# TheoCoombes/ClipCap

Measured on AMD Instinct MI355X. Metric: train samples/sec (512-d prefix, 40-tok caption), higher is better.
Workload: dtype bf16; 1 GPU; BASELINE configs[1]: TransformerMapper(8L,P=L=10,H=8)+frozen GPT-2-small; per_gpu_batch=256, global_batch=256, encoder_dim=512, train_language_model=False, parallelism=dp1

## Files before the change

clipcap_amd/csrc/attention.hip:

```cpp
#include "kernels.h"

namespace CC_NS {

__device__ __forceinline__ void load_head_rows(float* dst, int hdp, const act_t* src, size_t ld, int S, int hd) {
    const int c8n = hd >> 3;
    for (int idx = threadIdx.x; idx < S * c8n; idx += blockDim.x) {
        const int r = idx / c8n, c = idx % c8n;
        float f[8];
        act_ld8(src + (size_t)r * ld + c * 8, f);
        float* d = dst + r * hdp + c * 8;
        *reinterpret_cast<float4*>(d) = make_float4(f[0], f[1], f[2], f[3]);
        *reinterpret_cast<float4*>(d + 4) = make_float4(f[4], f[5], f[6], f[7]);
    }
}

template <auto Kernel, class... Args>
static void attn_launch(dim3 grid, dim3 block, size_t sh, hipStream_t st, const Args&... args) {
    if (sh > 64 * 1024) (void)hipFuncSetAttribute((const void*)Kernel, hipFuncAttributeMaxDynamicSharedMemorySize, (int)sh);
    hipLaunchKernelGGL(Kernel, grid, block, sh, st, args...);
}
#define ATTN_LADDER(LAUNCH) { if (drop.thresh) { LAUNCH(true, true); } else if (causal) { LAUNCH(true, false); } else { LAUNCH(false, false); } }

__device__ __forceinline__ unsigned attn_drop_idx(int b, int H, int h, int S, int q, int k) { return ((unsigned)(b * H + h) * S + q) * S + k; }
template <bool CAUSAL>
// ... 443 lines not shown
#pragma unroll
        for (int r = 0; r < 16; r++) acc[r] = 0.f;
        if (kind == 0) {
            const int jn = CAUSAL ? blk + 1 : NBLK;
            for (int j = 0; j < jn; j++)
#pragma unroll
                for (int t = 0; t < 2; t++) {
                    const op16x8 a_h = frag_row_p(Dh + (blk * 32 + l31) * LDP + j * 32, t, half), a_l = frag_row_p(Dl + (blk * 32 + l31) * LDP + j * 32, t, half);
                    const op16x8 b_h = frag_tr_p<LD>(Kh + j * 32 * LD, nb, t, lane), b_l = frag_tr_p<LD>(Kl + j * 32 * LD, nb, t, lane);
                    CC_MFMA3(a_h, a_l, b_h, b_l, acc)
                }
        } else {
            const op16_t* Ah = kind == 1 ? Dh : Ph, *Al = kind == 1 ? Dl : Pl, *Bh = kind == 1 ? Qh : Oh, *Bl = kind == 1 ? Ql : Ol;
            for (int i = CAUSAL ? blk : 0; i < NBLK; i++)
#pragma unroll
                for (int t = 0; t < 2; t++) {
                    const op16x8 a_h = frag_tr_p<LDP>(Ah + i * 32 * LDP, blk, t, lane), a_l = frag_tr_p<LDP>(Al + i * 32 * LDP, blk, t, lane);
                    const op16x8 b_h = frag_tr_p<LD>(Bh + i * 32 * LD, nb, t, lane), b_l = frag_tr_p<LD>(Bl + i * 32 * LD, nb, t, lane);
                    CC_MFMA3(a_h, a_l, b_h, b_l, acc)
                }
        }
        const int d = nb * 32 + l31;
        if (img) {
            const int odd = lane & 1;
            op16_t* r3 = reinterpret_cast<op16_t*>(dqkv) + (size_t)b * S * 9 * D + kind * D + h * HD + (d & ~1);
#pragma unroll
            for (int rp = 0; rp < 8; rp++) {
                const float v0 = acc[2 * rp], v1 = acc[2 * rp + 1];
                const float got = __shfl_xor(odd ? v0 : v1, 1, 64);
                const float a0 = odd ? got : v0, a1 = odd ? v1 : got;
                const int row = blk * 32 + ((2 * rp) & 3) + 8 * ((2 * rp) >> 2) + 4 * half + odd;
                const unsigned hi = pack2op(a0, a1);
                float h0, h1;
                unpack2(hi, h0, h1);
                const unsigned lo = pack2op(a0 - h0, a1 - h1);
                if (row < S) {
                    op16_t* o3 = r3 + (size_t)row * 9 * D;
                    *reinterpret_cast<unsigned*>(o3) = hi;
                    *reinterpret_cast<unsigned*>(o3 + 3 * D) = hi;
                    *reinterpret_cast<unsigned*>(o3 + 6 * D) = lo;
                }
            }
        } else {
            float* o1 = dqkv + (size_t)b * S * rs + kind * D + h * HD + d;
#pragma unroll
            for (int r = 0; r < 16; r++) {
                const int row = blk * 32 + (r & 3) + 8 * (r >> 2) + 4 * half;
                if (row < S) o1[(size_t)row * rs] = acc[r];
            }
        }
    }
    __syncthreads();
    }
}
template <int HD, int NBLK>
static int attn_bwd_m3_launch(const float* qkv, const float* dout, const float* lse, int B, int S, int H, bool causal, float* dqkv, hipStream_t st,
                              Drop drop, int img) {
    typedef AttM3<HD, NBLK> G;
    const float scale = 1.0f / sqrtf((float)HD);
    static int ncu = 0;
    if (!ncu) {
        int dev = 0;
        hipDeviceProp_t pr;
        if (hipGetDevice(&dev) != hipSuccess || hipGetDeviceProperties(&pr, dev) != hipSuccess) return CC_ERR_STATE;
        ncu = pr.multiProcessorCount;
    }
    const int per_cu = (int)((size_t)160 * 1024 / G::lds);
    const dim3 grid(min(B * H, ncu * max(1, per_cu))), blk(64 * G::NW);
    if (drop.thresh && !causal) return CC_ERR_SHAPE;
#define CC_L(C, DR) attn_launch<k_attn_bwd_m3<HD, NBLK, C, DR>>(grid, blk, G::lds, st, qkv, dout, lse, B, S, H, scale, dqkv, drop, img)
    ATTN_LADDER(CC_L)
#undef CC_L
    return hipGetLastError() == hipSuccess ? CC_OK : CC_ERR_LAUNCH;
}
static bool attn_x3mfma_on();
static bool attn_bwd_m3_ok(int S, int hd) { return attn_x3mfma_on() && (hd == 64 || hd == 96) && S > 0 && S <= 64; }
static bool attn_x3mfma_on() {
    static const bool on = !(cc_lab_env("CC_ATTN_X3MFMA") && atoi(cc_lab_env("CC_ATTN_X3MFMA")) == 0) && !cc_lab_env("CC_ATTN_F32MFMA");
    return on;
}
#endif

#if CC_OP != 2
template <int HD, bool CAUSAL, bool DROP = false>
__global__ __launch_bounds__(256, HD == 64 ? 3 : 2) void k_attn_fwd_mfma(const op16_t* __restrict__ qkv, int B, int S, int H, float scale,
                                                       op16_t* __restrict__ out, float* __restrict__ lse_out, Drop drop = Drop()) {
    constexpr int KK = HD / 16, NB = HD / 32, C8 = HD / 8;
    __shared__ __attribute__((aligned(16))) op16_t vsm[4][32 * AttLd<HD>::v];
    const int lane = threadIdx.x & 63, wave = threadIdx.x >> 6;
    const int nqb = (S + 31) >> 5;
    const int item = blockIdx.x * 4 + wave;
    if (item >= B * H * nqb) return;
    const int qb = item % nqb, h = (item / nqb) % H, b = item / (nqb * H);
    const int D = H * HD;
    const size_t rs = (size_t)3 * D;
    const op16_t* base = qkv + (size_t)b * S * rs + h * HD;
    const int half = lane >> 5, q = qb * 32 + (lane & 31);
    op16_t* vs = vsm[wave];

    op16x8 qf[KK];
#pragma unroll
    for (int kk = 0; kk < KK; kk++) {
        qf[kk] = load_frag(base + (size_t)min(q, S - 1) * rs + kk * 16 + half * 8, q < S);
    }
    f32x16 o[NB];
    acc_zero(o);
    float m = -INFINITY, l = 0.f;
    const int nkb = CAUSAL ? qb + 1 : nqb;
    uint4 kq[KK], vq[HD / 16];
    auto fetch = [&](int kb, uint4 (&kd)[KK], uint4 (&vd)[HD / 16]) {
        const int key = kb * 32 + (lane & 31);
#pragma unroll
        for (int kk = 0; kk < KK; kk++) {
            kd[kk] = *reinterpret_cast<const uint4*>(base + D + (size_t)min(key, S - 1) * rs + kk * 16 + half * 8);
            if (key >= S) kd[kk] = make_uint4(0, 0, 0, 0);
        }
#pragma unroll
        for (int c = 0; c < HD / 16; c++) {
            const int idx = lane + 64 * c;
            const int vk = idx / C8, vc = idx % C8;
            vd[c] = *reinterpret_cast<const uint4*>(base + 2 * D + (size_t)min(kb * 32 + vk, S - 1) * rs + vc * 8);
            if (kb * 32 + vk >= S) vd[c] = make_uint4(0, 0, 0, 0);
        }
    };
    fetch(0, kq, vq);
    for (int kb = 0; kb < nkb; kb++) {
        uint4 kn[KK], vn[HD / 16];
        fetch(kb + 1, kn, vn);
        f32x16 s;
        acc_zero(s);
#pragma unroll
        for (int kk = 0; kk < KK; kk++) s = CC_MFMA_32x32x16(__builtin_bit_cast(op16x8, kq[kk]), qf[kk], s);
#pragma unroll
        for (int c = 0; c < HD / 16; c++) {
            const int idx = lane + 64 * c;
            *reinterpret_cast<uint4*>(vs + (idx / C8) * AttLd<HD>::v + (idx % C8) * 8) = vq[c];
        }
        float mx = -INFINITY;
#pragma unroll
        for (int r = 0; r < 16; r++) {
            const int kr = kb * 32 + c_row(r, half);
            const bool ok = kr < S && (!CAUSAL || kr <= q);
            s[r] = ok ? s[r] * scale : -INFINITY;
            mx = fmaxf(mx, s[r]);
        }
        mx = fmaxf(mx, __shfl_xor(mx, 32, 64));
        const float m_new = fmaxf(m, mx);
        const float alpha = (m == -INFINITY) ? 0.f : __expf(m - m_new);
        float p[16], ps = 0.f;
#pragma unroll
        for (int r = 0; r < 16; r++) {
            p[r] = (m_new == -INFINITY) ? 0.f : __expf(s[r] - m_new);
            ps += p[r];
        }
        ps += __shfl_xor(ps, 32, 64);
        l = l * alpha + ps;
        m = m_new;
#pragma unroll
        for (int nb = 0; nb < NB; nb++)
#pragma unroll
            for (int r = 0; r < 16; r++) o[nb][r] *= alpha;
        if (DROP) {
            const unsigned rowbase = attn_drop_idx(b, H, h, S, min(q, S - 1), 0);
#pragma unroll
            for (int r = 0; r < 16; r++) p[r] *= drop_mul(drop, rowbase + min(kb * 32 + c_row(r, half), S - 1));
        }
        op16x8 pf[2];
#pragma unroll
        for (int t = 0; t < 2; t++) pf[t] = pack_frag(p + t * 8);
#pragma unroll
        for (int t = 0; t < 2; t++)
#pragma unroll
            for (int nb = 0; nb < NB; nb++) o[nb] = CC_MFMA_32x32x16(frag_tr<HD>(vs, nb, t, lane), pf[t], o[nb]);
#pragma unroll
        for (int kk = 0; kk < KK; kk++) kq[kk] = kn[kk];
#pragma unroll
        for (int c = 0; c < HD / 16; c++) vq[c] = vn[c];
    }
    if (q < S) {
        const float inv = l > 0.f ? 1.f / l : 0.f;
        op16_t* orow = out + ((size_t)b * S + q) * D + h * HD;
        store_acc_row<NB, true>(orow, o, half, inv);
        if (half == 0 && lse_out) lse_out[((size_t)b * H + h) * S + q] = m + __logf(l);
    }
}

template <int HD>
static int attn_fwd_mfma_launch(const op16_t* qkv, int B, int S, int H, bool causal, op16_t* out, float* lse, hipStream_t st, Drop drop) {
    const int items = B * H * ((S + 31) / 32);
    const float scale = 1.0f / sqrtf((float)HD);
    if (drop.thresh && !causal) return CC_ERR_SHAPE;
#define CC_L(C, DR) attn_launch<k_attn_fwd_mfma<HD, C, DR>>(dim3((items + 3) / 4), dim3(256), 0, st, qkv, B, S, H, scale, out, lse, drop)
    ATTN_LADDER(CC_L)
#undef CC_L
    return hipGetLastError() == hipSuccess ? CC_OK : CC_ERR_LAUNCH;
}


template <int HD, bool CAUSAL, bool DROP = false>
__global__ __launch_bounds__(256, HD == 64 ? 2 : 1) void k_attn_bwd_dkv(const op16_t* __restrict__ qkv, const op16_t* __restrict__ dout,
                                                      const float* __restrict__ lse, const float* __restrict__ delta, int B, int S, int H,
                                                      float scale, op16_t* __restrict__ dqkv, Drop drop = Drop()) {
    constexpr int KK = HD / 16, NB = HD / 32;
    __shared__ __attribute__((aligned(16))) op16_t qsm[4][32 * AttLd<HD>::v];
    __shared__ __attribute__((aligned(16))) op16_t dsm[4][32 * AttLd<HD>::v];
    __shared__ __attribute__((aligned(16))) float ldsm[4][64];
    const int lane = threadIdx.x & 63, wave = threadIdx.x >> 6;
    const int nblk = (S + 31) >> 5;
    const int item = blockIdx.x * 4 + wave;
    if (item >= B * H * nblk) return;
    const int j = item % nblk, h = (item / nblk) % H, b = item / (nblk * H);
    const int D = H * HD;
    const size_t rs = (size_t)3 * D;
    const op16_t* base = qkv + (size_t)b * S * rs + h * HD;
    const op16_t* dbase = dout + (size_t)b * S * D + h * HD;
    const float* lrow = lse + ((size_t)b * H + h) * S;
    const float* drow = delta + ((size_t)b * H + h) * S;
    const int half = lane >> 5, key = j * 32 + (lane & 31);
    op16x8 kf[KK], vf[KK];
#pragma unroll
    for (int kk = 0; kk < KK; kk++) {
        kf[kk] = load_frag(base + D + (size_t)min(key, S - 1) * rs + kk * 16 + half * 8, key < S);
        vf[kk] = load_frag(base + 2 * D + (size_t)min(key, S - 1) * rs + kk * 16 + half * 8, key < S);
    }
    f32x16 dk[NB], dv[NB];
#pragma unroll
    for (int nb = 0; nb < NB; nb++)
#pragma unroll
        for (int r = 0; r < 16; r++) { dk[nb][r] = 0.f; dv[nb][r] = 0.f; }
    const int i0 = CAUSAL ? j : 0;
    op16x8 qf[KK], df[KK];
    {
        const int qa = i0 * 32 + (lane & 31);
#pragma unroll
        for (int kk = 0; kk < KK; kk++) {
            qf[kk] = load_frag(base + (size_t)min(qa, S - 1) * rs + kk * 16 + half * 8, qa < S);
            df[kk] = load_frag(dbase + (size_t)min(qa, S - 1) * D + kk * 16 + half * 8, qa < S);
        }
    }
    for (int i = i0; i < nblk; i++) {
        op16x8 qn[KK], dn[KK];
        {
            const int qa = (i + 1) * 32 + (lane & 31);
#pragma unroll
            for (int kk = 0; kk < KK; kk++) {
                qn[kk] = load_frag(base + (size_t)min(qa, S - 1) * rs + kk * 16 + half * 8, qa < S);
                dn[kk] = load_frag(dbase + (size_t)min(qa, S - 1) * D + kk * 16 + half * 8, qa < S);
            }
        }
        f32x16 s, dp;
#pragma unroll
        for (int r = 0; r < 16; r++) { s[r] = 0.f; dp[r] = 0.f; }
#pragma unroll
        for (int kk = 0; kk < KK; kk++) {
            s = CC_MFMA_32x32x16(qf[kk], kf[kk], s);
            dp = CC_MFMA_32x32x16(df[kk], vf[kk], dp);
            *reinterpret_cast<op16x8*>(qsm[wave] + (lane & 31) * AttLd<HD>::v + kk * 16 + half * 8) = qf[kk];
            *reinterpret_cast<op16x8*>(dsm[wave] + (lane & 31) * AttLd<HD>::v + kk * 16 + half * 8) = df[kk];
        }
        {
            const int qq = min(i * 32 + (lane & 31), S - 1);
            ldsm[wave][lane] = half ? drow[qq] : lrow[qq];
        }
        float lq[16], dq_[16];
#pragma unroll
        for (int g4 = 0; g4 < 4; g4++) {
            const float4 a = *reinterpret_cast<const float4*>(&ldsm[wave][4 * half + 8 * g4]);
            const float4 b = *reinterpret_cast<const float4*>(&ldsm[wave][32 + 4 * half + 8 * g4]);
            lq[g4 * 4 + 0] = a.x; lq[g4 * 4 + 1] = a.y; lq[g4 * 4 + 2] = a.z; lq[g4 * 4 + 3] = a.w;
            dq_[g4 * 4 + 0] = b.x; dq_[g4 * 4 + 1] = b.y; dq_[g4 * 4 + 2] = b.z; dq_[g4 * 4 + 3] = b.w;
        }
        float p[16], ds[16];
#pragma unroll
        for (int r = 0; r < 16; r++) {
            const int qr = i * 32 + c_row(r, half);
            const bool ok = attn_live<CAUSAL>(qr, key, S);
// ... 60 lines not shown
        float x[8], y[8];
        unpack8(__builtin_bit_cast(uint4, dof[kk]), x);
        unpack8(__builtin_bit_cast(uint4, of), y);
#pragma unroll
        for (int e = 0; e < 8; e++) my_delta += x[e] * y[e];
    }
    my_delta += __shfl_xor(my_delta, 32, 64);
    if (half == 0 && q < S) delta[((size_t)b * H + h) * S + q] = my_delta;
    f32x16 dq[NB];
#pragma unroll
    for (int nb = 0; nb < NB; nb++)
#pragma unroll
        for (int r = 0; r < 16; r++) dq[nb][r] = 0.f;
    const int jend = CAUSAL ? i + 1 : nblk;
    op16x8 kf[KK], vf[KK];
    {
        const int key = lane & 31;
#pragma unroll
        for (int kk = 0; kk < KK; kk++) {
            kf[kk] = load_frag(base + D + (size_t)min(key, S - 1) * rs + kk * 16 + half * 8, key < S);
            vf[kk] = load_frag(base + 2 * D + (size_t)min(key, S - 1) * rs + kk * 16 + half * 8, key < S);
        }
    }
    for (int j = 0; j < jend; j++) {
        op16x8 kn[KK], vn[KK];
        {
            const int key = (j + 1) * 32 + (lane & 31);
#pragma unroll
            for (int kk = 0; kk < KK; kk++) {
                kn[kk] = load_frag(base + D + (size_t)min(key, S - 1) * rs + kk * 16 + half * 8, key < S);
                vn[kk] = load_frag(base + 2 * D + (size_t)min(key, S - 1) * rs + kk * 16 + half * 8, key < S);
            }
        }
        f32x16 st, dpt;
#pragma unroll
        for (int r = 0; r < 16; r++) { st[r] = 0.f; dpt[r] = 0.f; }
#pragma unroll
        for (int kk = 0; kk < KK; kk++) {
            st = CC_MFMA_32x32x16(kf[kk], qf[kk], st);
            dpt = CC_MFMA_32x32x16(vf[kk], dof[kk], dpt);
            *reinterpret_cast<op16x8*>(ksm[wave] + (lane & 31) * AttLd<HD>::v + kk * 16 + half * 8) = kf[kk];
        }
        float ds[16];
#pragma unroll
        for (int r = 0; r < 16; r++) {
            const int kr = j * 32 + c_row(r, half);
            const bool ok = kr < S && q < S && (!CAUSAL || kr <= q);
            const float p = ok ? __expf(st[r] * scale - my_lse) : 0.f;
            const float mk = DROP ? drop_mul(drop, attn_drop_idx(b, H, h, S, min(q, S - 1), min(kr, S - 1))) : 1.0f;
            ds[r] = p * (mk * dpt[r] - my_delta) * scale;
        }
        const op16x8 dsf[2] = {pack_frag(ds), pack_frag(ds + 8)};
#pragma unroll
        for (int t = 0; t < 2; t++)
#pragma unroll
            for (int nb = 0; nb < NB; nb++)
                dq[nb] = CC_MFMA_32x32x16(frag_tr<HD>(ksm[wave], nb, t, lane), dsf[t], dq[nb]);
#pragma unroll
        for (int kk = 0; kk < KK; kk++) { kf[kk] = kn[kk]; vf[kk] = vn[kk]; }
    }
    if (q < S) {
        op16_t* orow = dqkv + ((size_t)b * S + q) * rs + h * HD;
        store_acc_row<NB>(orow, dq, half);
    }
}

#ifndef CC_ATTN_FUSED_OCC
#define CC_ATTN_FUSED_OCC 2
#endif
template <int LD, int ROWS = 32>
__device__ __forceinline__ op16x8 frag_tr_ld(const op16_t* blk, int nb, int t, int lane) {
    typedef __attribute__((ext_vector_type(4))) short s16x4_t;
    typedef __attribute__((address_space(3))) s16x4_t* lp_t;
    const int half = lane >> 5, j = lane & 15, dsub = (lane >> 4) & 1;
    const int r0 = 16 * t + 4 * half + (j >> 2);
    const op16_t* col = blk + nb * 32 + 16 * dsub + 4 * (j & 3);
    const op16_t* p = col + (ROWS < 32 ? min(r0, ROWS - 1) : r0) * LD;
    const op16_t* ph = col + (ROWS < 32 ? min(r0 + 8, ROWS - 1) : r0 + 8) * LD;
    const s16x4_t lo = __builtin_amdgcn_ds_read_tr16_b64_v4i16((lp_t)p);
    const s16x4_t hi = __builtin_amdgcn_ds_read_tr16_b64_v4i16((lp_t)ph);
    typedef __attribute__((ext_vector_type(8))) short s16x8_t;
    const s16x8_t v = {lo[0], lo[1], lo[2], lo[3], hi[0], hi[1], hi[2], hi[3]};
    return __builtin_bit_cast(op16x8, v);
}

template <int HD>
__device__ __forceinline__ void attn_store_tile(op16_t* T, const f32x16 (&acc)[HD / 32], op16_t* gblock, size_t gstride, int rows_left, int lane) {
    constexpr int LD = AttLd<HD>::v, C8 = HD / 8;
    const int half = lane >> 5, l31 = lane & 31;
#pragma unroll
    for (int nb = 0; nb < HD / 32; nb++)
#pragma unroll
        for (int g = 0; g < 4; g++)
            *reinterpret_cast<uint2*>(T + l31 * LD + nb * 32 + 8 * g + 4 * half) =
                make_uint2(pack2op(acc[nb][g * 4 + 0], acc[nb][g * 4 + 1]), pack2op(acc[nb][g * 4 + 2], acc[nb][g * 4 + 3]));
#pragma unroll
    for (int it = 0; it < C8 / 2; it++) {
        const int idx = lane + 64 * it, row = idx / C8, chunk = idx % C8;
        const uint4 v = *reinterpret_cast<const uint4*>(T + row * LD + chunk * 8);
        if (row < rows_left) *reinterpret_cast<uint4*>(gblock + (size_t)row * gstride + chunk * 8) = v;
    }
}

template <int HD, bool CAUSAL, bool DROP, int NBLK, int OCC, int DR = 32>
__global__ __launch_bounds__(256, OCC) void k_attn_bwd_fused(const op16_t* __restrict__ qkv, const op16_t* __restrict__ dout, const op16_t* __restrict__ o,
                                                             const float* __restrict__ lse, int B, int S, int H, float scale,
                                                             op16_t* __restrict__ dqkv, Drop drop = Drop()) {
    constexpr int KK = HD / 16, NB = HD / 32, LD = AttLd<HD>::v;
    constexpr bool SPARE = LD >= HD + 32;
    constexpr int LT = SPARE ? LD : 32;
    __shared__ __attribute__((aligned(16))) op16_t ksm[4][32 * LD];
    __shared__ __attribute__((aligned(16))) op16_t qsm[4][32 * LD];
    __shared__ __attribute__((aligned(16))) op16_t dsm[4][32 * LD];
    static_assert(DR == 32 || (!SPARE && NBLK == 1), "the short dS^T tile is for the single-block form with its own tile");
    __shared__ __attribute__((aligned(16))) op16_t dtx[SPARE ? 1 : 4][SPARE ? 8 : DR * 32];
    __shared__ __attribute__((aligned(16))) float ldsm[4][NBLK][64];
    const int lane = threadIdx.x & 63, wave = threadIdx.x >> 6;
    const int item = blockIdx.x * 4 + wave;
    if (item >= B * H) return;
    const int h = item % H, b = item / H;
    const int D = H * HD;
    const size_t rs = (size_t)3 * D;
    const op16_t* base = qkv + (size_t)b * S * rs + h * HD;
    const op16_t* dbase = dout + (size_t)b * S * D + h * HD;
    const op16_t* obase = o + (size_t)b * S * D + h * HD;
    const float* lrow = lse + ((size_t)b * H + h) * S;
    const int half = lane >> 5, l31 = lane & 31;
    const int coff = half * 8;
    op16_t* dtm = SPARE ? ksm[wave] + HD : dtx[SPARE ? 0 : wave];

    op16x8 qf[KK], dof[KK], kf[KK], vf[KK];
    auto load_q = [&](int i) {
        const int q = i * 32 + l31, qc = min(q, S - 1);
#pragma unroll
        for (int kk = 0; kk < KK; kk++) {
            qf[kk] = load_frag(base + (size_t)qc * rs + kk * 16 + coff, q < S);
            dof[kk] = load_frag(dbase + (size_t)qc * D + kk * 16 + coff, q < S);
        }
    };
    auto load_k = [&](int j) {
        const int key = j * 32 + l31, kc = min(key, S - 1);
#pragma unroll
        for (int kk = 0; kk < KK; kk++) {
            kf[kk] = load_frag(base + D + (size_t)kc * rs + kk * 16 + coff, key < S);
            vf[kk] = load_frag(base + 2 * D + (size_t)kc * rs + kk * 16 + coff, key < S);
        }
    };
    load_k(0);
    load_q(0);
#pragma unroll
    for (int i = 0; i < NBLK; i++) {
        const int q = i * 32 + l31, qc = min(q, S - 1);
        float acc = 0.f;
#pragma unroll
        for (int kk = 0; kk < KK; kk++) {
            const op16x8 df = load_frag(dbase + (size_t)qc * D + kk * 16 + coff, q < S);
            const op16x8 of = load_frag(obase + (size_t)qc * D + kk * 16 + coff, q < S);
            float x[8], y[8];
            unpack8(__builtin_bit_cast(uint4, df), x);
            unpack8(__builtin_bit_cast(uint4, of), y);
#pragma unroll
            for (int e = 0; e < 8; e++) acc += x[e] * y[e];
        }
        acc += __shfl_xor(acc, 32, 64);
        ldsm[wave][i][lane] = half ? acc : lrow[qc];
    }
    f32x16 dq[NBLK][NB];

#pragma unroll
    for (int j = 0; j < NBLK; j++) {
        const int key = j * 32 + l31;
#pragma unroll
        for (int kk = 0; kk < KK; kk++) *reinterpret_cast<op16x8*>(ksm[wave] + l31 * LD + kk * 16 + coff) = kf[kk];
        f32x16 dk[NB], dv[NB];
#pragma unroll
        for (int nb = 0; nb < NB; nb++)
#pragma unroll
            for (int r = 0; r < 16; r++) { dk[nb][r] = 0.f; dv[nb][r] = 0.f; }
#pragma unroll
        for (int i = 0; i < NBLK; i++) {
            if (CAUSAL && i < j) continue;
            const int ifirst = CAUSAL ? j : 0;
            if (!(j > 0 && i == ifirst && i == NBLK - 1)) {
#pragma unroll
// ... 892 lines not shown
```

clipcap_amd/csrc/layernorm.hip:

```cpp
#include "kernels.h"

namespace CC_NS {

constexpr int LN_MAXV = 8;
#define LN_NV(D, LAUNCH, ...) { if ((D) <= 256) LAUNCH(1, ##__VA_ARGS__); else if ((D) <= 512) LAUNCH(2, ##__VA_ARGS__); else if ((D) <= 768) LAUNCH(3, ##__VA_ARGS__); else if ((D) <= 1024) LAUNCH(4, ##__VA_ARGS__); else LAUNCH(LN_MAXV, ##__VA_ARGS__); }
__device__ __forceinline__ int ln_col(int lane, int it) { return lane * 4 + it * 256; }

template <int NV>
__global__ __launch_bounds__(256) void k_ln_fwd(const float* __restrict__ x, int ldx, const int* __restrict__ row_map,
                                                const float* __restrict__ gamma, const float* __restrict__ beta,
                                                act_t* __restrict__ y, float* __restrict__ y32, float* __restrict__ mean,
                                                float* __restrict__ rstd, int rows, int D, float eps, int img) {
    constexpr int R = NV <= 4 ? 2 : 1;
    const int lane = threadIdx.x & 63;
    const int row0 = (blockIdx.x * 4 + (threadIdx.x >> 6)) * R;
    if (row0 >= rows) return;
    float4 v[R][NV], g[NV], bt[NV];
#pragma unroll
    for (int r = 0; r < R; r++) {
        const int row = min(row0 + r, rows - 1);
        const float* xr = x + (size_t)(row_map ? row_map[row] : row) * ldx;
#pragma unroll
        for (int it = 0; it < NV; it++) {
            const int c = ln_col(lane, it);
            v[r][it] = c < D ? *reinterpret_cast<const float4*>(xr + c) : make_float4(0, 0, 0, 0);
        }
    }
#pragma unroll
    for (int it = 0; it < NV; it++) {
        const int c = ln_col(lane, it);
        g[it] = c < D ? *reinterpret_cast<const float4*>(gamma + c) : make_float4(0, 0, 0, 0);
        bt[it] = c < D ? *reinterpret_cast<const float4*>(beta + c) : make_float4(0, 0, 0, 0);
    }
    float mu[R], rs[R];
#pragma unroll
    for (int r = 0; r < R; r++) {
        float s = 0.f;
#pragma unroll
        for (int it = 0; it < NV; it++) s += v[r][it].x + v[r][it].y + v[r][it].z + v[r][it].w;
        mu[r] = wave_sum(s) / D;
        float q = 0.f;
#pragma unroll
        for (int it = 0; it < NV; it++) {
            const int c = ln_col(lane, it);
            if (c < D) {
                const float a = v[r][it].x - mu[r], b = v[r][it].y - mu[r], cc_ = v[r][it].z - mu[r], d = v[r][it].w - mu[r];
                q += a * a + b * b + cc_ * cc_ + d * d;
            }
        }
        rs[r] = rsqrtf(wave_sum(q) / D + eps);
    }
#pragma unroll
    for (int r = 0; r < R; r++) {
        const int row = row0 + r;
        if (row >= rows) break;
        if (lane == 0) {
            if (mean) mean[row] = mu[r];
            if (rstd) rstd[row] = rs[r];
        }
#pragma unroll
        for (int it = 0; it < NV; it++) {
            const int c = lane * 4 + it * 256;
            if (c < D) {
                const float o0 = (v[r][it].x - mu[r]) * rs[r] * g[it].x + bt[it].x, o1 = (v[r][it].y - mu[r]) * rs[r] * g[it].y + bt[it].y;
                const float o2 = (v[r][it].z - mu[r]) * rs[r] * g[it].z + bt[it].z, o3 = (v[r][it].w - mu[r]) * rs[r] * g[it].w + bt[it].w;
#if CC_OP == 2
                if (y && img) {
                    uint2 hi, lo;
                    x3_pair4(o0, o1, o2, o3, hi, lo);
                    op16_t* r3 = reinterpret_cast<op16_t*>(y) + (size_t)row * 3 * D + c;
                    *reinterpret_cast<uint2*>(r3) = hi;
                    *reinterpret_cast<uint2*>(r3 + D) = hi;
                    *reinterpret_cast<uint2*>(r3 + 2 * D) = lo;
                } else
#endif
                if (y) act_st4(y + (size_t)row * D + c, o0, o1, o2, o3);
                if (y32) *reinterpret_cast<float4*>(y32 + (size_t)row * D + c) = make_float4(o0, o1, o2, o3);
            }
        }
    }
}
int ln_fwd(const float* x, int ldx, const int* row_map, const float* gamma, const float* beta, Act yo, float* y32,
           float* mean, float* rstd, int rows, int D, hipStream_t st) {
    if (D > LN_MAXV * 256 || (D & 3) || (ldx & 3)) return CC_ERR_SHAPE;
    if (rows <= 0) return CC_OK;
    const int rpb = D <= 1024 ? 8 : 4;
    const dim3 gr((rows + rpb - 1) / rpb);
    act_t* const y = yo.p;
    const int img = yo.img ? 1 : 0;
    if (img && (!kX3 || yo.img != D)) return CC_ERR_STATE;
#define LN_FWD(NV) hipLaunchKernelGGL(k_ln_fwd<NV>, gr, dim3(256), 0, st, x, ldx, row_map, gamma, beta, y, y32, mean, rstd, rows, D, 1e-5f, img)
    LN_NV(D, LN_FWD)
#undef LN_FWD
    return CC_OK;
}

template <int NV, bool DG, int NW>
__global__ __launch_bounds__(NW * 64) void k_ln_bwd(const act_t* __restrict__ dy, const float* __restrict__ x, int ldx,
                                                const int* __restrict__ row_map, const float* __restrict__ mean,
                                                const float* __restrict__ rstd, const float* __restrict__ gamma,
                                                const float* __restrict__ dres, float* __restrict__ dx32,
                                                act_t* __restrict__ dx16, float* __restrict__ dgamma, float* __restrict__ dbeta,
                                                float* __restrict__ dcol, int rows, int D, Drop dmask, int img, float* __restrict__ part) {
    extern __shared__ __attribute__((aligned(16))) float ln_red[];
    const int lane = threadIdx.x & 63, wave = threadIdx.x >> 6;
    float4 pg[DG ? NV : 1], pb[DG ? NV : 1], pc[DG ? NV : 1];
#pragma unroll
    for (int it = 0; it < (DG ? NV : 1); it++) pg[it] = pb[it] = pc[it] = make_float4(0, 0, 0, 0);
    float4 gmv[NV];
#pragma unroll
    for (int it = 0; it < NV; it++) {
        const int c = ln_col(lane, it);
        gmv[it] = c < D ? *reinterpret_cast<const float4*>(gamma + c) : make_float4(0, 0, 0, 0);
    }
    struct RowIn { act_raw4 d[NV]; float4 xv[NV], rr[NV]; float mu, rs; size_t xr; };
    auto fetch = [&](int row, RowIn& r) {
        r.xr = (size_t)(row_map ? row_map[row] : row) * ldx;
        r.mu = mean[row]; r.rs = rstd[row];
#pragma unroll
        for (int it = 0; it < NV; it++) {
            const int c = ln_col(lane, it);
            if (c < D) {
                r.d[it] = act_ldraw4(dy + (size_t)row * D + c);
                r.xv[it] = *reinterpret_cast<const float4*>(x + r.xr + c);
                r.rr[it] = dres ? *reinterpret_cast<const float4*>(dres + r.xr + c) : make_float4(0, 0, 0, 0);
            }
        }
    };
    const int rstep = gridDim.x * NW;
    int row = blockIdx.x * NW + wave;
    RowIn cur;
    if (row < rows) fetch(row, cur);
    for (; row < rows; row += rstep) {
        RowIn nxt;
        const bool more = DG && row + rstep < rows;
        if constexpr (DG) { if (more) fetch(row + rstep, nxt); }
        const size_t xr = cur.xr;
        const float mu = cur.mu, rs = cur.rs;
        float4 g[NV], xh[NV], rr[NV];
        float s1 = 0.f, s2 = 0.f;
#pragma unroll
        for (int it = 0; it < NV; it++) {
            const int c = ln_col(lane, it);
            if (c < D) {
                float d0, d1, d2, d3;
                act_unpack4(cur.d[it], d0, d1, d2, d3);
                const float4 xv = cur.xv[it];
                const float4 gm = gmv[it];
                rr[it] = cur.rr[it];
                xh[it] = make_float4((xv.x - mu) * rs, (xv.y - mu) * rs, (xv.z - mu) * rs, (xv.w - mu) * rs);
                g[it] = make_float4(d0 * gm.x, d1 * gm.y, d2 * gm.z, d3 * gm.w);
                s1 += g[it].x + g[it].y + g[it].z + g[it].w;
                s2 += g[it].x * xh[it].x + g[it].y * xh[it].y + g[it].z * xh[it].z + g[it].w * xh[it].w;
                if constexpr (DG) {
                    pg[it].x += d0 * xh[it].x; pg[it].y += d1 * xh[it].y; pg[it].z += d2 * xh[it].z; pg[it].w += d3 * xh[it].w;
                    pb[it].x += d0; pb[it].y += d1; pb[it].z += d2; pb[it].w += d3;
                }
            }
        }
        const float m1 = wave_sum(s1) / D, m2 = wave_sum(s2) / D;
#pragma unroll
        for (int it = 0; it < NV; it++) {
            const int c = ln_col(lane, it);
            if (c < D) {
                float4 o = make_float4(rs * (g[it].x - m1 - xh[it].x * m2), rs * (g[it].y - m1 - xh[it].y * m2),
                                       rs * (g[it].z - m1 - xh[it].z * m2), rs * (g[it].w - m1 - xh[it].w * m2));
                o.x += rr[it].x; o.y += rr[it].y; o.z += rr[it].z; o.w += rr[it].w;
                *reinterpret_cast<float4*>(dx32 + xr + c) = o;
                if (dx16) {
                    if (dmask.thresh) {
                        const unsigned e = (unsigned)(xr + c);
                        float m0, m1, m2, m3;
                        drop_mul_pair(dmask, e, m0, m1);
                        drop_mul_pair(dmask, e + 2, m2, m3);
                        o.x *= m0; o.y *= m1; o.z *= m2; o.w *= m3;
                    }
                    const act_raw4 pk = act_pack4(o.x, o.y, o.z, o.w);
#if CC_OP == 2
                    if (img) {
                        uint2 hi, lo;
                        x3_pair4(o.x, o.y, o.z, o.w, hi, lo);
                        x3_store4(reinterpret_cast<op16_t*>(dx16) + 3 * (size_t)xr + c, D, hi, lo);
                    } else
#endif
                    act_straw4(dx16 + xr + c, pk);
                    if constexpr (DG) {
                        if (dcol) {
                            float r0, r1, r2, r3;
                            act_unpack4(pk, r0, r1, r2, r3);
                            pc[it].x += r0; pc[it].y += r1; pc[it].z += r2; pc[it].w += r3;
                        }
                    }
                }
            }
        }
        if constexpr (DG) { if (more) cur = nxt; } else { if (row + rstep < rows) fetch(row + rstep, cur); }
    }
    if constexpr (DG) {
        float* rg = ln_red;
        float* rb = ln_red + NW * D;
        float* pp = part + (size_t)blockIdx.x * (dcol ? 3 : 2) * D;
#pragma unroll
        for (int it = 0; it < NV; it++) {
            const int c = ln_col(lane, it);
            if (c < D) {
                *reinterpret_cast<float4*>(rg + wave * D + c) = pg[it];
                *reinterpret_cast<float4*>(rb + wave * D + c) = pb[it];
            }
        }
        __syncthreads();
        for (int c = threadIdx.x; c < D; c += NW * 64) {
            float sg = 0.f, sb = 0.f;
#pragma unroll
            for (int w = 0; w < NW; w++) { sg += rg[w * D + c]; sb += rb[w * D + c]; }
            pp[c] = sg;
            pp[D + c] = sb;
        }
        if (dcol) {
            __syncthreads();
#pragma unroll
            for (int it = 0; it < NV; it++) {
                const int c = ln_col(lane, it);
                if (c < D) *reinterpret_cast<float4*>(rg + wave * D + c) = pc[it];
            }
            __syncthreads();
            for (int c = threadIdx.x; c < D; c += NW * 64) {
                float sc = 0.f;
#pragma unroll
                for (int w = 0; w < NW; w++) sc += rg[w * D + c];
                pp[2 * D + c] = sc;
            }
        }
    }
}
int ln_bwd(const act_t* dy, const float* x, int ldx, const int* row_map, const float* mean, const float* rstd,
           const float* gamma, const float* dres, float* dx32, Act dxo, float* dgamma, float* dbeta, int rows, int D,
           Call& cx, float* dcol, Drop dmask) {
    const hipStream_t st = cx.st;
    act_t* const dx16 = dxo.p;
    if (D > LN_MAXV * 256 || (D & 3) || (ldx & 3) || (dcol && (!dgamma || !dx16 || row_map)) || (dmask.thresh && (row_map || ldx != D)))
        return CC_ERR_SHAPE;
    if (rows <= 0) return CC_OK;
    const int nw = (dgamma && (size_t)16 * D * sizeof(float) <= 65536) ? 8 : 4;
    static const int dg_grid = []() { const char* e = cc_lab_env("CC_LNBWD_GRID"); return e ? atoi(e) : 256; }();
    const int nvec = dcol ? 3 : 2;
    const int grid = std::min((rows + nw - 1) / nw, dgamma ? std::max(1, std::min(dg_grid, (int)(RED_SCRATCH_FLOATS / ((size_t)nvec * D)))) : 8192);
    float* part = dgamma ? red_scratch(cx, (size_t)grid * nvec * D) : nullptr;
    if (dgamma && !part) return CC_ERR_STATE;
    const size_t sh = dgamma ? (size_t)2 * nw * D * sizeof(float) : 0;
    const int img = dxo.img ? 1 : 0;
    if (img && (!kX3 || dxo.img != D || ldx != D || dcol || dmask.thresh)) return CC_ERR_STATE;
#define LN_BWD(NV, DG, NW) hipLaunchKernelGGL((k_ln_bwd<NV, DG, NW>), dim3(grid), dim3(NW * 64), sh, st, dy, x, ldx, row_map, mean, rstd, gamma, dres, dx32, dx16, dgamma, dbeta, dcol, rows, D, dmask, img, part)
    if (dgamma && nw == 8) LN_NV(D, LN_BWD, true, 8) else if (dgamma) LN_NV(D, LN_BWD, true, 4) else LN_NV(D, LN_BWD, false, 4)
#undef LN_BWD
    if (!dgamma) return CC_OK;
    FoldOut o{};
    o.p[0] = dgamma; o.p[1] = dbeta; o.p[2] = dcol; o.m = D; o.k = nvec;
    return fold_partials(part, grid, nvec * D, 1, o, st);
}

}
```

Baseline: 22840 samples/s.

## Add whole-sequence per-head attention forward kernel for short sequences

Adds a specialized HD=64 forward attention kernel used when S<=64, where one wave handles an entire (batch, head) pair. It loads Q, K and V for both 32-row blocks once into registers, so K/V are reused across query blocks instead of being reloaded per query-block item. V is staged into LDS only on first use. It is enabled by default and can be turned off with an env var. The trade-offs are higher register pressure and fewer work items (B*H instead of B*H*nblk), which lowers parallelism.

Result: no change. 22770 samples/s (-0.3%).

```diff
diff --git a/clipcap_amd/csrc/attention.hip b/clipcap_amd/csrc/attention.hip
--- a/clipcap_amd/csrc/attention.hip
+++ b/clipcap_amd/csrc/attention.hip
@@ -652,11 +652,149 @@
     }
 }
 
+template <int KK>
+__device__ __forceinline__ f32x16 attn_fwd_scores(const uint4 (&kq)[KK], const op16x8 (&qf)[KK]) {
+    f32x16 s;
+    acc_zero(s);
+#pragma unroll
+    for (int kk = 0; kk < KK; kk++) s = CC_MFMA_32x32x16(__builtin_bit_cast(op16x8, kq[kk]), qf[kk], s);
+    return s;
+}
+template <int HD, bool CAUSAL, bool DROP>
+__device__ __forceinline__ void attn_fwd_softmax_pv(f32x16 s, const op16_t* vs, int kb, int q, int b, int H, int h, int S, int lane, float scale,
+                                                    const Drop& drop, float& m, float& l, f32x16 (&o)[HD / 32]) {
+    constexpr int NB = HD / 32;
+    const int half = lane >> 5;
+    float mx = -INFINITY;
+#pragma unroll
+    for (int r = 0; r < 16; r++) {
+        const int kr = kb * 32 + c_row(r, half);
+        const bool ok = kr < S && (!CAUSAL || kr <= q);
+        s[r] = ok ? s[r] * scale : -INFINITY;
+        mx = fmaxf(mx, s[r]);
+    }
+    mx = fmaxf(mx, __shfl_xor(mx, 32, 64));
+    const float m_new = fmaxf(m, mx);
+    const float alpha = (m == -INFINITY) ? 0.f : __expf(m - m_new);
+    float p[16], ps = 0.f;
+#pragma unroll
+    for (int r = 0; r < 16; r++) {
+        p[r] = (m_new == -INFINITY) ? 0.f : __expf(s[r] - m_new);
+        ps += p[r];
+    }
+    ps += __shfl_xor(ps, 32, 64);
+    l = l * alpha + ps;
+    m = m_new;
+#pragma unroll
+    for (int nb = 0; nb < NB; nb++)
+#pragma unroll
+        for (int r = 0; r < 16; r++) o[nb][r] *= alpha;
+    if (DROP) {
+        const unsigned rowbase = attn_drop_idx(b, H, h, S, min(q, S - 1), 0);
+#pragma unroll
+        for (int r = 0; r < 16; r++) p[r] *= drop_mul(drop, rowbase + min(kb * 32 + c_row(r, half), S - 1));
+    }
+    op16x8 pf[2];
+#pragma unroll
+    for (int t = 0; t < 2; t++) pf[t] = pack_frag(p + t * 8);
+#pragma unroll
+    for (int t = 0; t < 2; t++)
+#pragma unroll
+        for (int nb = 0; nb < NB; nb++) o[nb] = CC_MFMA_32x32x16(frag_tr<HD>(vs, nb, t, lane), pf[t], o[nb]);
+}
+template <int HD>
+__device__ __forceinline__ void attn_fwd_put_v(op16_t* vs, const uint4 (&vq)[HD / 16], int lane) {
+    constexpr int C8 = HD / 8;
+#pragma unroll
+    for (int c = 0; c < HD / 16; c++) {
+        const int idx = lane + 64 * c;
+        *reinterpret_cast<uint4*>(vs + (idx / C8) * AttLd<HD>::v + (idx % C8) * 8) = vq[c];
+    }
+}
+template <int HD>
+__device__ __forceinline__ void attn_fwd_store(op16_t* out, float* lse_out, const f32x16 (&o)[HD / 32], float m, float l, int b, int H, int h, int S, int q,
+                                               int half) {
+    if (q < S) {
+        const float inv = l > 0.f ? 1.f / l : 0.f;
+        op16_t* orow = out + ((size_t)b * S + q) * (H * HD) + h * HD;
+        store_acc_row<HD / 32, true>(orow, o, half, inv);
+        if (half == 0 && lse_out) lse_out[((size_t)b * H + h) * S + q] = m + __logf(l);
+    }
+}
+
+template <bool CAUSAL, bool DROP = false>
+__global__ __launch_bounds__(256, 3) void k_attn_fwd_whole(const op16_t* __restrict__ qkv, int B, int S, int H, float scale, op16_t* __restrict__ out,
+                                                           float* __restrict__ lse_out, Drop drop = Drop()) {
+    constexpr int HD = 64, KK = HD / 16, NB = HD / 32, C8 = HD / 8;
+    __shared__ __attribute__((aligned(16))) op16_t vsm[4][2][32 * AttLd<HD>::v];
+    const int lane = threadIdx.x & 63, wave = threadIdx.x >> 6;
+    const int item = blockIdx.x * 4 + wave;
+    if (item >= B * H) return;
+    const int h = item % H, b = item / H;
+    const int D = H * HD;
+    const size_t rs = (size_t)3 * D;
+    const op16_t* base = qkv + (size_t)b * S * rs + h * HD;
+    const int half = lane >> 5;
+    const int nblk = (S + 31) >> 5;
+
+    uint4 qf[2][KK], kf[2][KK], vf[2][HD / 16];
+#pragma unroll
+    for (int blk = 0; blk < 2; blk++) {
+        const int row = min(blk * 32 + (lane & 31), S - 1);
+#pragma unroll
+        for (int kk = 0; kk < KK; kk++) qf[blk][kk] = *reinterpret_cast<const uint4*>(base + (size_t)row * rs + kk * 16 + half * 8);
+#pragma unroll
+        for (int kk = 0; kk < KK; kk++) kf[blk][kk] = *reinterpret_cast<const uint4*>(base + D + (size_t)row * rs + kk * 16 + half * 8);
+#pragma unroll
+        for (int c = 0; c < HD / 16; c++) {
+            const int idx = lane + 64 * c;
+            vf[blk][c] = *reinterpret_cast<const uint4*>(base + 2 * D + (size_t)min(blk * 32 + idx / C8, S - 1) * rs + (idx % C8) * 8);
+        }
+    }
+#pragma unroll
+    for (int qb = 0; qb < 2; qb++) {
+        if (qb >= nblk) break;
+        const int q = qb * 32 + (lane & 31);
+        op16x8 qq[KK];
+#pragma unroll
+        for (int kk = 0; kk < KK; kk++) qq[kk] = __builtin_bit_cast(op16x8, q < S ? qf[qb][kk] : make_uint4(0, 0, 0, 0));
+        f32x16 o[NB];
+        acc_zero(o);
+        float m = -INFINITY, l = 0.f;
+#pragma unroll
+        for (int kb = 0; kb < 2; kb++) {
+            if (kb >= (CAUSAL ? qb + 1 : nblk)) break;
+            const bool first = qb == (CAUSAL ? kb : 0);
+            if (first) {
+#pragma unroll
+                for (int kk = 0; kk < KK; kk++)
+                    if (kb * 32 + (lane & 31) >= S) kf[kb][kk] = make_uint4(0, 0, 0, 0);
+#pragma unroll
+                for (int c = 0; c < HD / 16; c++)
+                    if (kb * 32 + (lane + 64 * c) / C8 >= S) vf[kb][c] = make_uint4(0, 0, 0, 0);
+            }
+            const f32x16 s = attn_fwd_scores(kf[kb], qq);
+            if (first) attn_fwd_put_v<HD>(vsm[wave][kb], vf[kb], lane);
+            attn_fwd_softmax_pv<HD, CAUSAL, DROP>(s, vsm[wave][kb], kb, q, b, H, h, S, lane, scale, drop, m, l, o);
+        }
+        attn_fwd_store<HD>(out, lse_out, o, m, l, b, H, h, S, q, half);
+    }
+}
+
 template <int HD>
 static int attn_fwd_mfma_launch(const op16_t* qkv, int B, int S, int H, bool causal, op16_t* out, float* lse, hipStream_t st, Drop drop) {
     const int items = B * H * ((S + 31) / 32);
     const float scale = 1.0f / sqrtf((float)HD);
     if (drop.thresh && !causal) return CC_ERR_SHAPE;
+    if constexpr (HD == 64) {
+        static const bool whole_on = []() { const char* e = cc_lab_env("CC_ATTN_FWD_WHOLE"); return !e || atoi(e) != 0; }();
+        if (S <= 64 && whole_on) {
+#define CC_L(C, DR) attn_launch<k_attn_fwd_whole<C, DR>>(dim3((B * H + 3) / 4), dim3(256), 0, st, qkv, B, S, H, scale, out, lse, drop)
+            ATTN_LADDER(CC_L)
+#undef CC_L
+            return hipGetLastError() == hipSuccess ? CC_OK : CC_ERR_LAUNCH;
+        }
+    }
 #define CC_L(C, DR) attn_launch<k_attn_fwd_mfma<HD, C, DR>>(dim3((items + 3) / 4), dim3(256), 0, st, qkv, B, S, H, scale, out, lse, drop)
     ATTN_LADDER(CC_L)
 #undef CC_L
```

## Stage attention fwd Q/K and output through swizzled LDS; pair rows in LN backward

Applied to the files above, without the earlier changes.

For head dim 64, the attention forward kernel now loads Q and K blocks with row-contiguous 16-byte loads, stages them through a swizzled LDS tile to form MFMA fragments, and writes the output through an LDS tile so global stores are coalesced. This targets strided per-lane global accesses, at the cost of extra LDS space and round trips that may reduce occupancy. LayerNorm backward without dgamma now has each wave process two rows per iteration with both loads issued up front and a higher occupancy hint. That path also drops the per-D NV dispatch in favour of LN_MAXV when pairing is off, which affects large D.

Result: no change. 22210 samples/s before, 22380 samples/s after (median of 6 runs) (+0.8%).

```diff
diff --git a/clipcap_amd/csrc/attention.hip b/clipcap_amd/csrc/attention.hip
--- a/clipcap_amd/csrc/attention.hip
+++ b/clipcap_amd/csrc/attention.hip
@@ -549,10 +549,33 @@
 #endif
 
 #if CC_OP != 2
-template <int HD, bool CAUSAL, bool DROP = false>
+template <int HD, bool MUL = false>
+__device__ __forceinline__ void attn_store_tile(op16_t* T, const f32x16 (&acc)[HD / 32], op16_t* gblock, size_t gstride, int rows_left, int lane, float f = 1.f) {
+    constexpr int LD = AttLd<HD>::v, C8 = HD / 8;
+    const int half = lane >> 5, l31 = lane & 31;
+#pragma unroll
+    for (int nb = 0; nb < HD / 32; nb++)
+#pragma unroll
+        for (int g = 0; g < 4; g++) {
+            const float a0 = MUL ? acc[nb][g * 4 + 0] * f : acc[nb][g * 4 + 0], a1 = MUL ? acc[nb][g * 4 + 1] * f : acc[nb][g * 4 + 1];
+            const float a2 = MUL ? acc[nb][g * 4 + 2] * f : acc[nb][g * 4 + 2], a3 = MUL ? acc[nb][g * 4 + 3] * f : acc[nb][g * 4 + 3];
+            *reinterpret_cast<uint2*>(T + l31 * LD + nb * 32 + 8 * g + 4 * half) = make_uint2(pack2op(a0, a1), pack2op(a2, a3));
+        }
+#pragma unroll
+    for (int it = 0; it < C8 / 2; it++) {
+        const int idx = lane + 64 * it, row = idx / C8, chunk = idx % C8;
+        const uint4 v = *reinterpret_cast<const uint4*>(T + row * LD + chunk * 8);
+        if (row < rows_left) *reinterpret_cast<uint4*>(gblock + (size_t)row * gstride + chunk * 8) = v;
+    }
+}
+
+template <int HD>
+__device__ __forceinline__ int attn_swz(int row, int chunk) { return row * AttLd<HD>::v + ((chunk ^ ((row >> 2) & 3)) * 8); }
+template <int HD, bool CAUSAL, bool DROP = false, int LINES = 2>
 __global__ __launch_bounds__(256, HD == 64 ? 3 : 2) void k_attn_fwd_mfma(const op16_t* __restrict__ qkv, int B, int S, int H, float scale,
                                                        op16_t* __restrict__ out, float* __restrict__ lse_out, Drop drop = Drop()) {
     constexpr int KK = HD / 16, NB = HD / 32, C8 = HD / 8;
+    constexpr bool TILE = LINES >= 1, LOADS = LINES == 2;
     __shared__ __attribute__((aligned(16))) op16_t vsm[4][32 * AttLd<HD>::v];
     const int lane = threadIdx.x & 63, wave = threadIdx.x >> 6;
     const int nqb = (S + 31) >> 5;
@@ -564,11 +587,39 @@
     const op16_t* base = qkv + (size_t)b * S * rs + h * HD;
     const int half = lane >> 5, q = qb * 32 + (lane & 31);
     op16_t* vs = vsm[wave];
+    op16_t* ks = nullptr;
+    if constexpr (LOADS) {
+        __shared__ __attribute__((aligned(16))) op16_t ksm[4][32 * AttLd<HD>::v];
+        ks = ksm[wave];
+    }
+    auto block_ld = [&](const op16_t* src, int r0, uint4 (&d)[HD / 16]) {
+#pragma unroll
+        for (int c = 0; c < HD / 16; c++) {
+            const int idx = lane + 64 * c;
+            const int rk = idx / C8, rc = idx % C8;
+            d[c] = *reinterpret_cast<const uint4*>(src + (size_t)min(r0 + rk, S - 1) * rs + rc * 8);
+            if (r0 + rk >= S) d[c] = make_uint4(0, 0, 0, 0);
+        }
+    };
+    auto tile_st = [&](op16_t* T, const uint4 (&d)[HD / 16]) {
+#pragma unroll
+        for (int c = 0; c < HD / 16; c++) {
+            const int idx = lane + 64 * c;
+            *reinterpret_cast<uint4*>(T + attn_swz<HD>(idx / C8, idx % C8)) = d[c];
+        }
+    };
+    auto tile_frag = [&](const op16_t* T, int kk) { return __builtin_bit_cast(op16x8, *reinterpret_cast<const uint4*>(T + attn_swz<HD>(lane & 31, 2 * kk + half))); };
 
     op16x8 qf[KK];
-#pragma unroll
-    for (int kk = 0; kk < KK; kk++) {
-        qf[kk] = load_frag(base + (size_t)min(q, S - 1) * rs + kk * 16 + half * 8, q < S);
+    if constexpr (LOADS) {
+        uint4 qd[HD / 16];
+        block_ld(base, qb * 32, qd);
+        tile_st(vs, qd);
+#pragma unroll
+        for (int kk = 0; kk < KK; kk++) qf[kk] = tile_frag(vs, kk);
+    } else {
+#pragma unroll
+        for (int kk = 0; kk < KK; kk++) qf[kk] = load_frag(base + (size_t)min(q, S - 1) * rs + kk * 16 + half * 8, q < S);
     }
     f32x16 o[NB];
     acc_zero(o);
@@ -576,11 +627,15 @@
     const int nkb = CAUSAL ? qb + 1 : nqb;
     uint4 kq[KK], vq[HD / 16];
     auto fetch = [&](int kb, uint4 (&kd)[KK], uint4 (&vd)[HD / 16]) {
-        const int key = kb * 32 + (lane & 31);
-#pragma unroll
-        for (int kk = 0; kk < KK; kk++) {
-            kd[kk] = *reinterpret_cast<const uint4*>(base + D + (size_t)min(key, S - 1) * rs + kk * 16 + half * 8);
-            if (key >= S) kd[kk] = make_uint4(0, 0, 0, 0);
+        if constexpr (LOADS) {
+            block_ld(base + D, kb * 32, kd);
+        } else {
+            const int key = kb * 32 + (lane & 31);
+#pragma unroll
+            for (int kk = 0; kk < KK; kk++) {
+                kd[kk] = *reinterpret_cast<const uint4*>(base + D + (size_t)min(key, S - 1) * rs + kk * 16 + half * 8);
+                if (key >= S) kd[kk] = make_uint4(0, 0, 0, 0);
+            }
         }
 #pragma unroll
         for (int c = 0; c < HD / 16; c++) {
@@ -596,8 +651,14 @@
         fetch(kb + 1, kn, vn);
         f32x16 s;
         acc_zero(s);
-#pragma unroll
-        for (int kk = 0; kk < KK; kk++) s = CC_MFMA_32x32x16(__builtin_bit_cast(op16x8, kq[kk]), qf[kk], s);
+        if constexpr (LOADS) {
+            tile_st(ks, kq);
+#pragma unroll
+            for (int kk = 0; kk < KK; kk++) s = CC_MFMA_32x32x16(tile_frag(ks, kk), qf[kk], s);
+        } else {
+#pragma unroll
+            for (int kk = 0; kk < KK; kk++) s = CC_MFMA_32x32x16(__builtin_bit_cast(op16x8, kq[kk]), qf[kk], s);
+        }
 #pragma unroll
         for (int c = 0; c < HD / 16; c++) {
             const int idx = lane + 64 * c;
@@ -644,10 +705,10 @@
 #pragma unroll
         for (int c = 0; c < HD / 16; c++) vq[c] = vn[c];
     }
+    const float inv = l > 0.f ? 1.f / l : 0.f;
+    if constexpr (TILE) attn_store_tile<HD, true>(vs, o, out + ((size_t)b * S + qb * 32) * D + h * HD, D, S - qb * 32, lane, inv);
     if (q < S) {
-        const float inv = l > 0.f ? 1.f / l : 0.f;
-        op16_t* orow = out + ((size_t)b * S + q) * D + h * HD;
-        store_acc_row<NB, true>(orow, o, half, inv);
+        if constexpr (!TILE) store_acc_row<NB, true>(out + ((size_t)b * S + q) * D + h * HD, o, half, inv);
         if (half == 0 && lse_out) lse_out[((size_t)b * H + h) * S + q] = m + __logf(l);
     }
 }
@@ -657,8 +718,22 @@
     const int items = B * H * ((S + 31) / 32);
     const float scale = 1.0f / sqrtf((float)HD);
     if (drop.thresh && !causal) return CC_ERR_SHAPE;
-#define CC_L(C, DR) attn_launch<k_attn_fwd_mfma<HD, C, DR>>(dim3((items + 3) / 4), dim3(256), 0, st, qkv, B, S, H, scale, out, lse, drop)
+#define CC_L(C, DR) attn_launch<k_attn_fwd_mfma<HD, C, DR, CC_LINES>>(dim3((items + 3) / 4), dim3(256), 0, st, qkv, B, S, H, scale, out, lse, drop)
+#ifdef CC_EXPERIMENTS
+    if constexpr (HD == 64) {
+        static const int lines = []() { const char* e = cc_lab_env("CC_ATTN_FWD_LINES"); return e ? atoi(e) : 2; }();
+#define CC_LINES 1
+        if (lines == 1) ATTN_LADDER(CC_L) else
+#undef CC_LINES
+#define CC_LINES 0
+        if (lines == 0) ATTN_LADDER(CC_L)
+#undef CC_LINES
+        if (lines == 0 || lines == 1) return hipGetLastError() == hipSuccess ? CC_OK : CC_ERR_LAUNCH;
+    }
+#endif
+#define CC_LINES (HD == 64 ? 2 : 0)
     ATTN_LADDER(CC_L)
+#undef CC_LINES
 #undef CC_L
     return hipGetLastError() == hipSuccess ? CC_OK : CC_ERR_LAUNCH;
 }
@@ -885,24 +960,6 @@
     typedef __attribute__((ext_vector_type(8))) short s16x8_t;
     const s16x8_t v = {lo[0], lo[1], lo[2], lo[3], hi[0], hi[1], hi[2], hi[3]};
     return __builtin_bit_cast(op16x8, v);
-}
-
-template <int HD>
-__device__ __forceinline__ void attn_store_tile(op16_t* T, const f32x16 (&acc)[HD / 32], op16_t* gblock, size_t gstride, int rows_left, int lane) {
-    constexpr int LD = AttLd<HD>::v, C8 = HD / 8;
-    const int half = lane >> 5, l31 = lane & 31;
-#pragma unroll
-    for (int nb = 0; nb < HD / 32; nb++)
-#pragma unroll
-        for (int g = 0; g < 4; g++)
-            *reinterpret_cast<uint2*>(T + l31 * LD + nb * 32 + 8 * g + 4 * half) =
-                make_uint2(pack2op(acc[nb][g * 4 + 0], acc[nb][g * 4 + 1]), pack2op(acc[nb][g * 4 + 2], acc[nb][g * 4 + 3]));
-#pragma unroll
-    for (int it = 0; it < C8 / 2; it++) {
-        const int idx = lane + 64 * it, row = idx / C8, chunk = idx % C8;
-        const uint4 v = *reinterpret_cast<const uint4*>(T + row * LD + chunk * 8);
-        if (row < rows_left) *reinterpret_cast<uint4*>(gblock + (size_t)row * gstride + chunk * 8) = v;
-    }
 }
 
 template <int HD, bool CAUSAL, bool DROP, int NBLK, int OCC, int DR = 32>
diff --git a/clipcap_amd/csrc/layernorm.hip b/clipcap_amd/csrc/layernorm.hip
--- a/clipcap_amd/csrc/layernorm.hip
+++ b/clipcap_amd/csrc/layernorm.hip
@@ -95,8 +95,8 @@
     return CC_OK;
 }
 
-template <int NV, bool DG, int NW>
-__global__ __launch_bounds__(NW * 64) void k_ln_bwd(const act_t* __restrict__ dy, const float* __restrict__ x, int ldx,
+template <int NV, bool DG, int NW, bool PAIR>
+__global__ __launch_bounds__(NW * 64, (PAIR && NV == 3) ? 4 : 1) void k_ln_bwd(const act_t* __restrict__ dy, const float* __restrict__ x, int ldx,
                                                 const int* __restrict__ row_map, const float* __restrict__ mean,
                                                 const float* __restrict__ rstd, const float* __restrict__ gamma,
                                                 const float* __restrict__ dres, float* __restrict__ dx32,
@@ -127,14 +127,7 @@
             }
         }
     };
-    const int rstep = gridDim.x * NW;
-    int row = blockIdx.x * NW + wave;
-    RowIn cur;
-    if (row < rows) fetch(row, cur);
-    for (; row < rows; row += rstep) {
-        RowIn nxt;
-        const bool more = DG && row + rstep < rows;
-        if constexpr (DG) { if (more) fetch(row + rstep, nxt); }
+    auto reduce = [&](const RowIn& cur) {
         const size_t xr = cur.xr;
         const float mu = cur.mu, rs = cur.rs;
         float4 g[NV], xh[NV], rr[NV];
@@ -194,7 +187,28 @@
                 }
             }
         }
-        if constexpr (DG) { if (more) cur = nxt; } else { if (row + rstep < rows) fetch(row + rstep, cur); }
+    };
+    const int rstep = gridDim.x * NW;
+    int row = blockIdx.x * NW + wave;
+    if constexpr (PAIR) {
+        static_assert(!DG && NV <= 4, "the pair form is the plain form's");
+        for (; 2 * row < rows; row += rstep) {
+            RowIn a, b;
+            fetch(2 * row, a);
+            fetch(min(2 * row + 1, rows - 1), b);
+            reduce(a);
+            if (2 * row + 1 < rows) reduce(b);
+        }
+    } else {
+        RowIn cur;
+        if (row < rows) fetch(row, cur);
+        for (; row < rows; row += rstep) {
+            RowIn nxt;
+            const bool more = DG && row + rstep < rows;
+            if constexpr (DG) { if (more) fetch(row + rstep, nxt); }
+            reduce(cur);
+            if constexpr (DG) { if (more) cur = nxt; } else { if (row + rstep < rows) fetch(row + rstep, cur); }
+        }
     }
     if constexpr (DG) {
         float* rg = ln_red;
@@ -244,14 +258,27 @@
     const int nw = (dgamma && (size_t)16 * D * sizeof(float) <= 65536) ? 8 : 4;
     static const int dg_grid = []() { const char* e = cc_lab_env("CC_LNBWD_GRID"); return e ? atoi(e) : 256; }();
     const int nvec = dcol ? 3 : 2;
-    const int grid = std::min((rows + nw - 1) / nw, dgamma ? std::max(1, std::min(dg_grid, (int)(RED_SCRATCH_FLOATS / ((size_t)nvec * D)))) : 8192);
+#ifdef CC_EXPERIMENTS
+    static const bool pairs = []() { const char* e = cc_lab_env("CC_LNBWD_ROWS"); return !(e && atoi(e) == 1); }();
+#else
+    constexpr bool pairs = true;
+#endif
+    const bool pair = !dgamma && pairs && D <= 1024;
+    const int rpb = pair ? 2 * nw : nw;
+    const int grid = std::min((rows + rpb - 1) / rpb, dgamma ? std::max(1, std::min(dg_grid, (int)(RED_SCRATCH_FLOATS / ((size_t)nvec * D)))) : 8192);
     float* part = dgamma ? red_scratch(cx, (size_t)grid * nvec * D) : nullptr;
     if (dgamma && !part) return CC_ERR_STATE;
     const size_t sh = dgamma ? (size_t)2 * nw * D * sizeof(float) : 0;
     const int img = dxo.img ? 1 : 0;
     if (img && (!kX3 || dxo.img != D || ldx != D || dcol || dmask.thresh)) return CC_ERR_STATE;
-#define LN_BWD(NV, DG, NW) hipLaunchKernelGGL((k_ln_bwd<NV, DG, NW>), dim3(grid), dim3(NW * 64), sh, st, dy, x, ldx, row_map, mean, rstd, gamma, dres, dx32, dx16, dgamma, dbeta, dcol, rows, D, dmask, img, part)
-    if (dgamma && nw == 8) LN_NV(D, LN_BWD, true, 8) else if (dgamma) LN_NV(D, LN_BWD, true, 4) else LN_NV(D, LN_BWD, false, 4)
+#define LN_BWD(NV, DG, NW, PAIR) hipLaunchKernelGGL((k_ln_bwd<NV, DG, NW, PAIR>), dim3(grid), dim3(NW * 64), sh, st, dy, x, ldx, row_map, mean, rstd, gamma, dres, dx32, dx16, dgamma, dbeta, dcol, rows, D, dmask, img, part)
+    if (dgamma && nw == 8) LN_NV(D, LN_BWD, true, 8, false) else if (dgamma) LN_NV(D, LN_BWD, true, 4, false)
+    else if (pair) { if (D <= 256) LN_BWD(1, false, 4, true); else if (D <= 512) LN_BWD(2, false, 4, true); else if (D <= 768) LN_BWD(3, false, 4, true); else LN_BWD(4, false, 4, true); }
+#ifdef CC_EXPERIMENTS
+    else LN_NV(D, LN_BWD, false, 4, false)
+#else
+    else LN_BWD(LN_MAXV, false, 4, false);
+#endif
 #undef LN_BWD
     if (!dgamma) return CC_OK;
     FoldOut o{};
```
